# lightkurve/lightkurve

Measured on AMD Instinct MI355X. Metric: frequencies*targets/sec (Lomb-Scargle, ls_method='fast' (reference default): extirpolation + FFT) + BLS periods*targets/sec; max-power rel-err, higher is better.
Workload: dtype f64

## Files before the change

lightkurve_amd/csrc/lsfast.hip:

```cpp
#include <cmath>
#include <cstdlib>
#include <type_traits>
#include <vector>

#include "lk_common.hpp"
#include "ls_epilogue.hpp"

namespace lk {

typedef double lk_d2v __attribute__((ext_vector_type(2)));

constexpr int SPREAD_W = 1024;
constexpr int SPREAD_WW = 256;

struct FastStats {
    double wsum, ybar, YY, t0;
    double yws;
    double wmax;
    double vmax;
};

__device__ __forceinline__ void cadence_weights(const double *__restrict__ y, const double *__restrict__ dy, int64_t i,
                                                double wsum, double ybar, double &w, double &wy) {
    const double d = dy ? dy[i] : 1.0;
// ... 479 lines not shown
        }
        if (gout)
            gout[((size_t)blockIdx.y << (m1 + m2)) + ((((size_t)(c >> twl) << m1) + k1) << twl) + (c & (tw - 1))] = cmul(v, w);
        else
            G[(size_t)k1 * N2 + c] = cmul(v, w);
        w = cmul(w, step);
    };
    block_fft<LA, LB, 1>(CT, lds2, load, store);
}

constexpr int PRUNED_CT = 16;

constexpr int LSF_CHUNK_HALF_GB = 3;

template <int LP>
__global__ __launch_bounds__(PRUNED_CT * (1 << ((LP + 1) / 2)), 2) void fft_cols_pruned_kernel(
    const double2 *__restrict__ grids, int m1, int m2, const int *__restrict__ rows_used, double2 *__restrict__ gout,
    const double *__restrict__ t, const double *__restrict__ y, const double *__restrict__ dy,
    const int64_t *__restrict__ n_off, const FastStats *__restrict__ stats, int b0, double f0, double df, int fit_mean,
    const int *__restrict__ tab16, int ntab16) {
    extern __shared__ __attribute__((aligned(16))) double2 lds2[];
    constexpr int LA = (LP + 1) / 2, LB = LP / 2, A = 1 << LA, Bq = 1 << LB, P = 1 << LP, LDT = Bq + 1, FST = A * LDT + 1;
    constexpr int CT = PRUNED_CT, NT = CT * A;
    const int N1 = 1 << m1, N2 = 1 << m2, Q = N1 >> LP;
    const double2 *G = grids + ((size_t)blockIdx.y << (m1 + m2));
    const size_t tstride = (size_t)CT << m1, gstride = (size_t)(N2 / CT) * tstride;
    double2 *O = gout + (size_t)blockIdx.y * gstride + (size_t)blockIdx.x * tstride;
    const int c0 = blockIdx.x * CT;
    const int lbt = blockIdx.y / 3, g = blockIdx.y % 3;
    const int ru = rows_used[lbt * 4 + g];
    const int tid = threadIdx.x;
    const int f = tid % CT, jk = tid / CT;
    const bool p1 = jk < Bq, p2 = jk < A;
    const double invN1 = 1.0 / (double)N1, invN = 1.0 / (double)((size_t)1 << (m1 + m2));
    double2 xin[A];
    if (tab16 != nullptr && rows_used[lbt * 4 + 3]) {
        double2 *acc = lds2;
        for (int e = tid; e < ru * CT; e += NT) acc[e] = make_double2(0.0, 0.0);
        __syncthreads();
        if (!(g == 1 && !fit_mean)) {
            const int b = b0 + lbt;
            const int64_t lo = n_off[b];
            const FastStats st = stats[b];
            const double fac = g == 2 ? 2.0 : 1.0, dff = df * fac, f0f = f0 * fac, dn = (double)((size_t)1 << (m1 + m2));
            const int nfft = 1 << (m1 + m2);
            const int *tlo = tab16 + ((size_t)b * 4 + (g == 2 ? 2 : 0)) * ntab16, *thi = tlo + ntab16;
            const int S = g == 2 ? 4 : 8, rpi = 64 / S;
            const int lane = tid & 63, wv = tid >> 6, rr = lane / S, k = lane - rr * S;
            const int rpw = (ru + NT / 64 - 1) / (NT / 64);
            const int r_end = min(ru, (wv + 1) * rpw);
            auto visit = [&](int r, double ti, double yi, double di) {
                const double tt = ti - st.t0;
                const double wi = (1.0 / (di * di)) / st.wsum, wyi = wi * (yi - st.ybar);
                double c = 1.0, sn = 0.0;
                if (f0f > 0.0) phase_factor(f0f, tt, c, sn);
                const double xp = tt * dn * dff;
                const Stencil4 sp = stencil4(xp < dn ? xp : fmod(xp, dn), nfft);
                const double amp = g == 0 ? wyi : wi, ar = amp * c, ai = amp * sn;
                const int cbase = (r << m2) + c0;
#pragma unroll
                for (int q = 0; q < 4; ++q) {
                    const unsigned col = (unsigned)(sp.i0 + q - cbase);
                    if (q < sp.n && col < (unsigned)CT) {
                        unsafeAtomicAdd(&acc[r * CT + col].x, ar * sp.wt[q]);
                        unsafeAtomicAdd(&acc[r * CT + col].y, ai * sp.wt[q]);
                    }
                }
            };
            constexpr int UN = 4;
            for (int rb = wv * rpw; rb < r_end; rb += UN * rpi) {
                int ii[UN], ih[UN];
#pragma unroll
                for (int u = 0; u < UN; ++u) {
                    const int r = rb + u * rpi + rr;
                    const int blk = (min(r, r_end - 1) << (m2 - 4)) + blockIdx.x;
                    ii[u] = tlo[blk] + k;
                    ih[u] = thi[blk + 1];
                }
#pragma unroll
                for (int u = 0; u < UN; ++u) {
                    asm volatile("" : "+v"(ii[u]), "+v"(ih[u]));
                    if (rb + u * rpi + rr >= r_end) ii[u] = ih[u] = 0;
                }
                double tv[UN], yv[UN], dv[UN];
#pragma unroll
                for (int u = 0; u < UN; ++u) {
                    const bool ok = ii[u] < ih[u];
                    const int64_t ix = lo + (ok ? ii[u] : 0);
                    tv[u] = t[ix];
                    yv[u] = y[ix];
                    dv[u] = dy ? dy[ix] : 1.0;
                }
#pragma unroll
                for (int u = 0; u < UN; ++u) {
                    const int r = rb + u * rpi + rr;
                    if (ii[u] < ih[u]) visit(r, tv[u], yv[u], dv[u]);
                    int i = ii[u] + S;
                    while (__any(i < ih[u])) {
                        if (i < ih[u]) visit(r, t[lo + i], y[lo + i], dy ? dy[lo + i] : 1.0);
                        i += S;
                    }
                }
            }
        }
        __syncthreads();
        if (p1) {
#pragma unroll
            for (int i = 0; i < A; ++i) {
                const int r = i * Bq + jk;
                xin[i] = r < ru ? acc[r * CT + f] : make_double2(0.0, 0.0);
            }
        }
        __syncthreads();
    } else if (p1) {
#pragma unroll
        for (int i = 0; i < A; ++i) {
            const int r = i * Bq + jk;
            xin[i] = r < ru ? G[(size_t)r * N2 + c0 + f] : make_double2(0.0, 0.0);
        }
    }
    auto root = [](double x) {
        double sn, cs;
        sincospi(2.0 * x, &sn, &cs);
        return make_double2(cs, sn);
    };
    const double2 wj = root((double)jk * invN1), wq = root((double)Bq * invN1);
    const double2 tw_j = root((double)jk / (double)P);
    const double2 wc = root((double)(c0 + f) * invN), stepc = root((double)((long long)(c0 + f) * Q * A) * invN);
    double2 wjs = make_double2(1.0, 0.0), wqs = wjs;
    double2 wout = root((double)((long long)(c0 + f) * Q * jk) * invN);
    for (int s = 0; s < Q; ++s) {
        if (p1) {
            double2 v[A];
            if (s == 0) {
#pragma unroll
                for (int i = 0; i < A; ++i) v[i] = xin[i];
            } else {
                double2 w = wjs;
#pragma unroll
                for (int i = 0; i < A; ++i) {
                    v[i] = cmul(xin[i], w);
                    w = cmul(w, wqs);
                }
            }
            reg_fft<LA>(v);
            double2 w = make_double2(1.0, 0.0);
            double2 *row = lds2 + (size_t)f * FST + jk;
#pragma unroll
            for (int ka = 0; ka < A; ++ka) {
                row[ka * LDT] = cmul(v[brev_c(ka, LA)], w);
                w = cmul(w, tw_j);
            }
        }
        __syncthreads();
        if (p2) {
            const double2 *row = lds2 + (size_t)f * FST + (size_t)jk * LDT;
            double2 u[Bq];
#pragma unroll
            for (int j = 0; j < Bq; ++j) u[j] = row[j];
            reg_fft<LB>(u);
            double2 w = wout;
#pragma unroll
            for (int kb = 0; kb < Bq; ++kb) {
                const int q = jk + A * kb;
                O[(size_t)(Q * q + s) * CT + f] = cmul(u[brev_c(kb, LB)], w);
                w = cmul(w, stepc);
            }
        }
        wjs = cmul(wjs, wj);
        wqs = cmul(wqs, wq);
        wout = cmul(wout, wc);
        __syncthreads();
    }
}

template <int LA, int LB>
__global__ __launch_bounds__(256) void fft_rows_reg_kernel(const double2 *__restrict__ grids, int m1, int RT, int nkeep,
                                                            double2 *__restrict__ spec) {
    extern __shared__ __attribute__((aligned(16))) double2 lds2[];
    constexpr int m2 = LA + LB;
    const int N2 = 1 << m2;
    const double2 *G = grids + ((size_t)blockIdx.y << (m1 + m2));
    double2 *S = spec + (size_t)blockIdx.y * nkeep;
    const int r0 = blockIdx.x * RT;
    auto load = [&](int f, int c) -> double2 { return G[(size_t)(r0 + f) * N2 + c]; };
    auto store = [&](int f, int k2, double2 v, int) {
        const long long k = (long long)(r0 + f) + ((long long)k2 << m1);
        if (k < nkeep) S[k] = v;
    };
    block_fft<LA, LB, 0>(RT, lds2, load, store);
}

struct PeakPart {
    double v;
    long long k;
};

__device__ __forceinline__ bool peak_better(double v2, long long k2, double v, long long k) {
    return k2 >= 0 && (k < 0 || v2 > v || (v2 == v && k2 < k));
}

template <int LA, int LB, int KB>
__global__ __launch_bounds__(512) void fft_rows_power_kernel(const double2 *__restrict__ grids, int m1, int RT,
                                                              const int64_t *__restrict__ n_off,
                                                              const FastStats *__restrict__ stats, int b0, double f0,
                                                              double df, int64_t M, int fit_mean, int norm,
                                                              const double *__restrict__ scale,
                                                              double *__restrict__ power, int tw,
                                                              PeakPart *__restrict__ peaks) {
    extern __shared__ __attribute__((aligned(16))) double2 lds2[];
    constexpr int m2 = LA + LB, A = 1 << LA;
    const int N2 = 1 << m2;
    const int twl = tw ? 31 - __clz(tw) : 0;
    const size_t tstride = tw ? ((size_t)tw << m1) : 0, gstride = (size_t)1 << (m1 + m2);
    const int lb = blockIdx.y, r0 = blockIdx.x * RT;
    double2 keep0[KB], keep1[KB], keep2[KB];
#pragma unroll
    for (int q = 0; q < KB; ++q) keep0[q] = keep1[q] = keep2[q] = make_double2(0.0, 0.0);
    auto transform = [&](int g, double2(&keep)[KB]) {
        const double2 *G = grids + (size_t)(lb * 3 + g) * gstride;
        auto load = [&](int f, int c) -> double2 {
            return tw ? G[(size_t)(c >> twl) * tstride + ((size_t)(r0 + f) << twl) + (c & (tw - 1))] : G[(size_t)(r0 + f) * N2 + c];
        };
        auto store = [&](int, int, double2 v, int kb) {
            if (kb < KB) keep[kb < KB ? kb : 0] = v;
        };
        if (tw)
            block_fft<LA, LB, 2>(RT, lds2, load, store, tw);
        else
            block_fft<LA, LB, 0>(RT, lds2, load, store);
    };
    transform(0, keep0);
    __syncthreads();
    if (fit_mean) transform(1, keep1);
    __syncthreads();
    transform(2, keep2);
    const int tid = threadIdx.x;
    double best_v = 0.0;
    long long best_k = -1;
    if (tid < RT * A) {
        const int ka = tid / RT, f = tid - ka * RT;
        const int b = b0 + lb;
        const FastStats st = stats[b];
        const double nn = (double)(n_off[b + 1] - n_off[b]);
        const double sc = scale ? scale[b] : 1.0;
        const int k1 = r0 + f;
        const double twopi = 6.283185307179586;
        double ph_c = 1.0, ph_s = 0.0, st_c = 1.0, st_s = 0.0;
        if (st.t0 != 0.0) {
            const long long kfirst = (long long)k1 + ((long long)ka << m1);
            sincos(twopi * st.t0 * (f0 + df * (double)kfirst), &ph_s, &ph_c);
            sincos(twopi * st.t0 * (df * (double)((long long)A << m1)), &st_s, &st_c);
        }
#pragma unroll
        for (int kb = 0; kb < KB; ++kb) {
            const long long k = (long long)k1 + ((long long)(ka + A * kb) << m1);
            if (k < M) {
                double2 a = keep0[kb], bq = keep1[kb], c2 = keep2[kb];
                if (st.t0 != 0.0) {
                    const double c = ph_c, s = ph_s;
                    a = make_double2(a.x * c - a.y * s, a.x * s + a.y * c);
                    bq = make_double2(bq.x * c - bq.y * s, bq.x * s + bq.y * c);
                    const double cc = c * c - s * s, ss = 2.0 * s * c;
                    c2 = make_double2(c2.x * cc - c2.y * ss, c2.x * ss + c2.y * cc);
                }
                const double pw = gls_power_sums(a.y, a.x, bq.y, bq.x, c2.y, c2.x, fit_mean, norm, st.YY, 0.5 * st.wsum, nn, sc);
                power[(size_t)b * (size_t)M + k] = pw;
                if (pw == pw && peak_better(pw, k, best_v, best_k)) {
                    best_v = pw;
                    best_k = k;
                }
            }
            const double nc = ph_c * st_c - ph_s * st_s, ns = ph_s * st_c + ph_c * st_s;
            ph_c = nc;
            ph_s = ns;
        }
    }
    if (peaks == nullptr) return;
#pragma unroll
    for (int o = 32; o > 0; o >>= 1) {
        const double v2 = __shfl_xor(best_v, o);
        const long long k2 = __shfl_xor(best_k, o);
        if (peak_better(v2, k2, best_v, best_k)) {
            best_v = v2;
            best_k = k2;
        }
    }
    if ((tid & 63) == 0)
        peaks[((size_t)lb * gridDim.x + blockIdx.x) * (blockDim.x >> 6) + (tid >> 6)] = PeakPart{best_v, best_k};
}

__device__ __forceinline__ double dpp_ror8(double x) {
    int lo = __double2loint(x), hi = __double2hiint(x);
    lo = __builtin_amdgcn_update_dpp(0, lo, 0x128, 0xF, 0xF, true);
    hi = __builtin_amdgcn_update_dpp(0, hi, 0x128, 0xF, 0xF, true);
    return __hiloint2double(hi, lo);
}

struct Rows512 {
    static constexpr int RT = 8;
    static constexpr int SK = 34;
    static constexpr int SF = 16 * SK + 4;
    static constexpr int NT = RT * 32;
    static constexpr size_t LDS_BYTES = (size_t)RT * SF * 8;
};

__global__ __launch_bounds__(Rows512::NT, 2) void fft_rows512_power_kernel(
    const double2 *__restrict__ grids, int m1, int ntargets, const int64_t *__restrict__ n_off,
    const FastStats *__restrict__ stats, int b0, double f0, double df, int64_t M, int fit_mean, int norm,
    const double *__restrict__ scale, double *__restrict__ power, PeakPart *__restrict__ peaks) {
    using R = Rows512;
    constexpr int RT = R::RT, SK = R::SK, SF = R::SF;
    extern __shared__ __attribute__((aligned(16))) double tile512[];
    const int tid = threadIdx.x;
    const size_t gstride = (size_t)1 << (m1 + 9);
    const int tiles_per_target = (1 << m1) / RT;
    const int jl = tid & 15, f1 = (tid >> 4) & (RT - 1), jh = tid >> 7, j = jl + 16 * jh;
    const int f2 = tid & 7, e = (tid >> 3) & 1, ka = tid >> 4;
    auto tile_base = [&](int T) {
        const int lbT = ntargets - 1 - T / tiles_per_target, r0T = (T % tiles_per_target) * RT;
        return grids + (size_t)lbT * 3 * gstride + ((size_t)jh << (m1 + 4)) + ((size_t)(r0T + f1) << 4) + jl;
    };
    double2 v[16];
    auto load = [&](const double2 *G) {
#pragma unroll
        for (int i = 0; i < 16; ++i) {
            const lk_d2v q = __builtin_nontemporal_load(reinterpret_cast<const lk_d2v *>(G + ((size_t)i << (m1 + 5))));
            v[i] = make_double2(q.x, q.y);
        }
    };
    double2 step1, step4;
    {
        double s, c;
        sincospi((double)j * (1.0 / 256.0), &s, &c);
        step1 = make_double2(c, s);
        sincospi((double)j * (1.0 / 64.0), &s, &c);
        step4 = make_double2(c, s);
    }
    double2 keep[3][4];
    double *row1 = tile512 + f1 * SF + j;
    const double *row2 = tile512 + f2 * SF + ka * SK + e;
    auto process = [&](auto Gc, auto refill) {
        constexpr int G = decltype(Gc)::value;
        __builtin_amdgcn_sched_barrier(0);
        reg_fft<4>(v);
        __builtin_amdgcn_sched_barrier(0);
        {
            double2 w = step1;
#pragma unroll
            for (int bb = 1; bb < 4; ++bb) {
#pragma unroll
                for (int a = 0; a < 4; ++a) v[brev_c(4 * a + bb, 4)] = cmul(v[brev_c(4 * a + bb, 4)], w);
                if (bb < 3) w = cmul(w, step1);
            }
        }
        __builtin_amdgcn_sched_barrier(0);
        {
            double2 w = step4;
#pragma unroll
            for (int a = 1; a < 4; ++a) {
#pragma unroll
                for (int bb = 0; bb < 4; ++bb) v[brev_c(4 * a + bb, 4)] = cmul(v[brev_c(4 * a + bb, 4)], w);
                if (a < 3) w = cmul(w, step4);
            }
        }
        __builtin_amdgcn_sched_barrier(0);
        double ure[16], uim[16];
#pragma unroll
        for (int k = 0; k < 16; ++k) row1[k * SK] = v[brev_c(k, 4)].x;
        __syncthreads();
#pragma unroll
        for (int jj = 0; jj < 16; ++jj) ure[jj] = row2[2 * jj];
        __syncthreads();
#pragma unroll
        for (int k = 0; k < 16; ++k) row1[k * SK] = v[brev_c(k, 4)].y;
        __builtin_amdgcn_sched_barrier(0);
        refill();
        __syncthreads();
#pragma unroll
        for (int jj = 0; jj < 16; ++jj) uim[jj] = row2[2 * jj];
        __builtin_amdgcn_sched_barrier(0);
        double2 s0[8], s1[8];
#pragma unroll
        for (int q = 0; q < 8; ++q) {
            s0[q] = make_double2(ure[2 * q], uim[2 * q]);
            s1[q] = make_double2(ure[2 * q + 1], uim[2 * q + 1]);
        }
        reg_fft<3>(s0);
        __builtin_amdgcn_sched_barrier(0);
        reg_fft<3>(s1);
        __builtin_amdgcn_sched_barrier(0);
        auto pval = [&](int kb) -> double2 {
            const double2 a = s0[brev_c(kb, 3)], bq = s1[brev_c(kb, 3)];
            double2 hsum;
            if (kb == 0)
                hsum = make_double2(a.x + bq.x, a.y + bq.y);
            else if (kb == 4)
                hsum = make_double2(a.x - bq.y, a.y + bq.x);
            else
                hsum = make_double2(a.x + (bq.x * R32C[2 * kb] - bq.y * R32S[2 * kb]),
                                    a.y + (bq.x * R32S[2 * kb] + bq.y * R32C[2 * kb]));
            if (kb == 0) return hsum;
            const double wc = e ? R32C[kb] : 1.0, ws = e ? R32S[kb] : 0.0;
            return make_double2(hsum.x * wc - hsum.y * ws, hsum.x * ws + hsum.y * wc);
        };
#pragma unroll
        for (int q = 0; q < 4; ++q) {
            const double2 plo = pval(q), phi = pval(q + 4);
            const double2 mine = e ? phi : plo, send = e ? plo : phi;
            keep[G][q] = make_double2(mine.x + dpp_ror8(send.x), mine.y + dpp_ror8(send.y));
            __builtin_amdgcn_sched_barrier(0);
        }
    };
    using I0 = std::integral_constant<int, 0>;
    using I1 = std::integral_constant<int, 1>;
    using I2 = std::integral_constant<int, 2>;
    const int T = blockIdx.x;
    const double2 *Gt = tile_base(T);
    load(Gt);
    {
        const int lb = ntargets - 1 - T / tiles_per_target, r0 = (T % tiles_per_target) * RT;
        process(I0{}, [&] { load(Gt + gstride); });
        __syncthreads();
        process(I1{}, [&] { load(Gt + 2 * gstride); });
        __syncthreads();
        process(I2{}, [] {});
        double best_v = 0.0;
        long long best_k = -1;
        {
            const int b = b0 + lb;
            const FastStats st = stats[b];
            const double nn = (double)(n_off[b + 1] - n_off[b]);
            const double sc = scale ? scale[b] : 1.0;
            const int k1 = r0 + f2;
            const double twopi = 6.283185307179586;
            double ph_c = 1.0, ph_s = 0.0, st_c = 1.0, st_s = 0.0;
            if (st.t0 != 0.0) {
                const long long kfirst = (long long)k1 + ((long long)(ka + 64 * e) << m1);
                sincos(twopi * st.t0 * (f0 + df * (double)kfirst), &ph_s, &ph_c);
                sincos(twopi * st.t0 * (df * (double)((long long)16 << m1)), &st_s, &st_c);
            }
#pragma unroll 1
            for (int q = 0; q < 4; ++q) {
                const long long k = (long long)k1 + ((long long)(ka + 16 * (4 * e + q)) << m1);
                if (k < M) {
                    double2 a = keep[0][0], bq = keep[1][0], c2 = keep[2][0];
                    if (st.t0 != 0.0) {
                        const double c = ph_c, s = ph_s;
                        a = make_double2(a.x * c - a.y * s, a.x * s + a.y * c);
                        bq = make_double2(bq.x * c - bq.y * s, bq.x * s + bq.y * c);
                        const double cc = c * c - s * s, ss = 2.0 * s * c;
                        c2 = make_double2(c2.x * cc - c2.y * ss, c2.x * ss + c2.y * cc);
                    }
                    const double pw = gls_power_sums(a.y, a.x, bq.y, bq.x, c2.y, c2.x, fit_mean, norm, st.YY, 0.5 * st.wsum, nn, sc);
                    power[(size_t)b * (size_t)M + k] = pw;
                    if (pw == pw && peak_better(pw, k, best_v, best_k)) {
                        best_v = pw;
                        best_k = k;
                    }
                }
                const double nc = ph_c * st_c - ph_s * st_s, ns = ph_s * st_c + ph_c * st_s;
                ph_c = nc;
                ph_s = ns;
#pragma unroll
                for (int g = 0; g < 3; ++g)
#pragma unroll
                    for (int r = 0; r < 3; ++r) keep[g][r] = keep[g][r + 1];
            }
        }
        if (peaks != nullptr) {
#pragma unroll
            for (int o = 32; o > 0; o >>= 1) {
                const double v2 = __shfl_xor(best_v, o);
                const long long k2 = __shfl_xor(best_k, o);
                if (peak_better(v2, k2, best_v, best_k)) {
                    best_v = v2;
                    best_k = k2;
                }
            }
            if ((tid & 63) == 0)
                peaks[((size_t)lb * tiles_per_target + (T % tiles_per_target)) * (R::NT / 64) + (tid >> 6)] = PeakPart{best_v, best_k};
        }
    }
}

__global__ __launch_bounds__(64) void lsf_peaks_kernel(const PeakPart *__restrict__ peaks, int nparts, int b0,
                                                        double *__restrict__ max_out, int64_t *__restrict__ arg_out) {
    const PeakPart *pp = peaks + (size_t)blockIdx.x * nparts;
    double v = 0.0;
    long long k = -1;
    for (int i = threadIdx.x; i < nparts; i += 64)
        if (peak_better(pp[i].v, pp[i].k, v, k)) {
            v = pp[i].v;
            k = pp[i].k;
        }
#pragma unroll
    for (int o = 32; o > 0; o >>= 1) {
        const double v2 = __shfl_xor(v, o);
        const long long k2 = __shfl_xor(k, o);
        if (peak_better(v2, k2, v, k)) {
            v = v2;
            k = k2;
        }
    }
    if (threadIdx.x == 0) {
        max_out[b0 + blockIdx.x] = k >= 0 ? v : NAN;
        arg_out[b0 + blockIdx.x] = (int64_t)k;
    }
}

__global__ __launch_bounds__(256) void lsf_scatter_multi_kernel(const double *__restrict__ t, const double *__restrict__ y,
                                                                 const double *__restrict__ dy,
                                                                 const int64_t *__restrict__ n_off,
                                                                 const FastStats *__restrict__ stats, int b0, double f0,
                                                                 double df, int nfft, int nterms,
                                                                 double2 *__restrict__ grids) {
    const int b = b0 + blockIdx.y;
    const int64_t lo = n_off[b];
    const int n = (int)(n_off[b + 1] - lo);
    const int i = blockIdx.x * 256 + threadIdx.x;
    if (i >= n) return;
    const FastStats st = stats[b];
    const double tt = t[lo + i] - st.t0;
    double2 *g0 = grids + (size_t)blockIdx.y * 3 * nterms * nfft;
    double wi, wyi;
    cadence_weights(y, dy, lo + i, st.wsum, st.ybar, wi, wyi);
    const Quantum Qy = make_quantum(st.vmax), Qw = make_quantum(st.wmax);
    for (int fac = 1; fac <= 2 * nterms; ++fac) {
        const double dff = df * (double)fac, f0f = f0 * (double)fac;
        double c = 1.0, s = 0.0;
        if (f0f > 0.0) phase_factor(f0f, tt, c, s);
        const Stencil4 sp = stencil4(fmod(tt * (double)nfft * dff, (double)nfft), nfft);
        extirpolate4(g0 + (size_t)(nterms + fac - 1) * nfft, sp, wi * c, wi * s, Qw);
        if (fac <= nterms) extirpolate4(g0 + (size_t)(fac - 1) * nfft, sp, wyi * c, wyi * s, Qy);
    }
}

template <int NT>
__global__ __launch_bounds__(256) void lsf_chi2_power_kernel(const double2 *__restrict__ spec,
                                                              const int64_t *__restrict__ n_off,
                                                              const FastStats *__restrict__ stats, int b0, double f0,
                                                              double df, int64_t M, int fit_mean, int norm,
                                                              const double *__restrict__ scale,
                                                              double *__restrict__ power) {
    const int b = b0 + blockIdx.y;
    const int64_t j = (int64_t)blockIdx.x * 256 + threadIdx.x;
    if (j >= M) return;
    const FastStats st = stats[b];
    const double2 *s0 = spec + (size_t)blockIdx.y * 3 * NT * M;
    Chi2Sums<NT> sums;
    const double twopi = 6.283185307179586;
#pragma unroll
    for (int m = 1; m <= 2 * NT; ++m) {
        double cph = 1.0, sph = 0.0;
        if (st.t0 != 0.0) sincos(twopi * st.t0 * (double)m * (f0 + df * (double)j), &sph, &cph);
        const double2 a = s0[(size_t)(NT + m - 1) * M + j];
        sums.Cw[m - 1] = a.x * cph - a.y * sph;
        sums.Sw[m - 1] = a.x * sph + a.y * cph;
        if (m <= NT) {
            const double2 y = s0[(size_t)(m - 1) * M + j];
            sums.Cy[m - 1] = y.x * cph - y.y * sph;
            sums.Sy[m - 1] = y.x * sph + y.y * cph;
        }
    }
    const double n = (double)(n_off[b + 1] - n_off[b]);
    power[(size_t)b * (size_t)M + j] =
        chi2_normalise(sums.solve_lu(st.yws, fit_mean), norm, st.YY, 0.5 * st.wsum, n, scale ? scale[b] : 1.0);
}

__global__ __launch_bounds__(256) void lsf_power_kernel(const double2 *__restrict__ spec,
                                                         const int64_t *__restrict__ n_off,
                                                         const FastStats *__restrict__ stats, int b0, double f0,
                                                         double df, int64_t M, int fit_mean, int norm,
                                                         const double *__restrict__ scale,
                                                         double *__restrict__ power) {
    const int b = b0 + blockIdx.y;
    const int64_t j = (int64_t)blockIdx.x * 256 + threadIdx.x;
    if (j >= M) return;
    const FastStats st = stats[b];
    const double2 *s0 = spec + (size_t)blockIdx.y * 3 * M;
    double2 a = s0[j], bq = s0[M + j], c2 = s0[2 * M + j];
    if (st.t0 != 0.0) {
        const double twopi = 6.283185307179586;
        double s, c;
        sincos(twopi * st.t0 * (f0 + df * (double)j), &s, &c);
        a = make_double2(a.x * c - a.y * s, a.x * s + a.y * c);
        bq = make_double2(bq.x * c - bq.y * s, bq.x * s + bq.y * c);
        sincos(twopi * st.t0 * (2.0 * f0 + 2.0 * df * (double)j), &s, &c);
        c2 = make_double2(c2.x * c - c2.y * s, c2.x * s + c2.y * c);
    }
    const double n = (double)(n_off[b + 1] - n_off[b]);
    power[(size_t)b * (size_t)M + j] = gls_power_sums(a.y, a.x, bq.y, bq.x, c2.y, c2.x, fit_mean, norm, st.YY,
                                                      0.5 * st.wsum, n, scale ? scale[b] : 1.0);
}

__global__ __launch_bounds__(256) void lsf_unquantize_kernel(double2 *__restrict__ grids, int m1, int m2,
                                                              const int *__restrict__ rows_used,
                                                              const FastStats *__restrict__ stats, int b0, int ngp, int n_wy) {
    const int lbt = blockIdx.y / ngp, g = blockIdx.y % ngp;
    if (rows_used && rows_used[lbt * 4 + 3]) return;
    const int ru = rows_used ? rows_used[lbt * 4 + g] : (1 << m1);
    const FastStats st = stats[b0 + lbt];
    const double q = make_quantum(g < n_wy ? st.vmax : st.wmax).q;
    if (!(q > 0.0)) return;
    const int N2 = 1 << m2;
    double2 *G = grids + ((size_t)blockIdx.y << (m1 + m2));
    for (int r = blockIdx.x * 8; r < min(blockIdx.x * 8 + 8, ru); ++r)
        for (int c = threadIdx.x; c < N2; c += 256) {
            const double2 v = G[(size_t)r * N2 + c];
            G[(size_t)r * N2 + c] = make_double2((double)__double_as_longlong(v.x) * q, (double)__double_as_longlong(v.y) * q);
        }
}

__global__ __launch_bounds__(256) void lsf_zero_kernel(double2 *__restrict__ grids, int m1, int m2,
                                                        const int *__restrict__ rows_used) {
    if (rows_used[(blockIdx.y / 3) * 4 + 3]) return;
    const int ru = rows_used[(blockIdx.y / 3) * 4 + (blockIdx.y % 3)];
    const int N2 = 1 << m2;
    double2 *G = grids + ((size_t)blockIdx.y << (m1 + m2));
    for (int r = blockIdx.x * 8; r < min(blockIdx.x * 8 + 8, ru); ++r)
        for (int c = threadIdx.x; c < N2; c += 256) G[(size_t)r * N2 + c] = make_double2(0.0, 0.0);
}

constexpr int COLS_TILE_PTS = 4096;

template <int LA, int LB>
static void launch_cols_t(lk_handle *h, int m2, int ngrids, double2 *grids, const int *rows_used, double2 *gout, int tw,
                          hipStream_t stream) {
    constexpr int A = 1 << LA, Bq = 1 << LB, n = A * Bq, LDT = Bq + 1, FST = A * LDT + 1;
    const int N2 = 1 << m2;
    const int CT = std::max(1, std::min(N2, std::min(COLS_TILE_PTS / n, 256 / std::max(A, Bq))));
    const int nt = ((CT * std::max(A, Bq) + 63) / 64) * 64;
    (void)want_lds(h, reinterpret_cast<const void *>(fft_cols_reg_kernel<LA, LB>), 160 * 1024);
    hipLaunchKernelGGL((fft_cols_reg_kernel<LA, LB>), dim3(N2 / CT, ngrids), dim3(nt), (size_t)CT * FST * 16, stream, grids,
                       m2, CT, rows_used, gout, tw);
}

static int tile_width(int m1, int m2) {
    const int la1 = (m1 + 1) / 2, lb1 = m1 / 2, n1 = 1 << m1;
    const int ct = std::max(1, std::min(1 << m2, std::min(COLS_TILE_PTS / n1, 256 / std::max(1 << la1, 1 << lb1))));
    const int bq2 = 1 << (m2 / 2);
    return std::min(ct, bq2);
}

template <int LA, int LB>
static void launch_rows_t(lk_handle *h, int m1, int ngrids, const double2 *grids, int nkeep, double2 *spec, hipStream_t stream) {
    constexpr int A = 1 << LA, Bq = 1 << LB, n = A * Bq, LDT = Bq + 1, FST = A * LDT + 1;
    const int N1 = 1 << m1;
    const int RT = std::max(1, std::min(N1, std::min(4096 / n, 256 / std::max(A, Bq))));
    const int nt = ((RT * std::max(A, Bq) + 63) / 64) * 64;
    (void)want_lds(h, reinterpret_cast<const void *>(fft_rows_reg_kernel<LA, LB>), 100 * 1024);
    hipLaunchKernelGGL((fft_rows_reg_kernel<LA, LB>), dim3(N1 / RT, ngrids), dim3(nt), (size_t)RT * FST * 16, stream,
                       grids, m1, RT, nkeep, spec);
}

struct FusedArgs {
    const int64_t *n_off;
    const FastStats *stats;
    int b0;
    double f0, df;
    int64_t M;
    int fit_mean, norm;
    const double *scale;
    double *power;
    PeakPart *peaks;
};

template <int LA, int LB>
static int rows_power_rt(int m1) {
    constexpr int A = 1 << LA, Bq = 1 << LB, n = A * Bq;
    return std::max(1, std::min(1 << m1, std::min(4096 / n, 256 / std::max(A, Bq))));
}

template <int LA, int LB, int KB>
static void launch_rows_power_t(lk_handle *h, int m1, int ntargets, const double2 *grids, const FusedArgs &a, int tw,
                                hipStream_t stream) {
    constexpr int A = 1 << LA, Bq = 1 << LB, LDT = Bq + 1, FST = A * LDT + 1;
    const int N1 = 1 << m1;
    const int RT = rows_power_rt<LA, LB>(m1);
    const int nt = ((RT * std::max(A, Bq) + 63) / 64) * 64;
    (void)want_lds(h, reinterpret_cast<const void *>(fft_rows_power_kernel<LA, LB, KB>), 160 * 1024);
    hipLaunchKernelGGL((fft_rows_power_kernel<LA, LB, KB>), dim3(N1 / RT, ntargets), dim3(nt), (size_t)RT * FST * 16,
                       stream, grids, m1, RT, a.n_off, a.stats, a.b0, a.f0, a.df, a.M, a.fit_mean, a.norm, a.scale,
                       a.power, tw, a.peaks);
}

static bool rows_power_available(int m1, int m2, int64_t M) {
    const int LA = (m2 + 1) / 2, Aa = 1 << LA;
    const long long k2need = (M + ((long long)1 << m1) - 1) >> m1;
    return m2 >= 4 && m2 <= 10 && (k2need + Aa - 1) / Aa <= 8;
}

#define LK_M2_SWITCH(m2, X) \
    switch (m2) {           \
        case 4: X(2, 2)     \
        case 5: X(3, 2)     \
        case 6: X(3, 3)     \
        case 7: X(4, 3)     \
        case 8: X(4, 4)     \
        case 9: X(5, 4)     \
        default: X(5, 5)    \
    }

static int rows_power_parts(int m1, int m2) {
#define LK_X(la, lb)                                                                                   \
    {                                                                                                  \
        const int rt = rows_power_rt<la, lb>(m1);                                                      \
        return ((1 << m1) / rt) * ((rt * std::max(1 << (la), 1 << (lb)) + 63) / 64);                   \
    }
    LK_M2_SWITCH(m2, LK_X)
#undef LK_X
}

static bool rows512_applies(int m1, int m2, int64_t M, int tw) {
    const long long k2need = (M + ((long long)1 << m1) - 1) >> m1;
    return m2 == 9 && tw == PRUNED_CT && m1 >= 3 && k2need <= 128;
}

static void launch_rows512(lk_handle *h, int m1, int ntargets, const double2 *grids, const FusedArgs &a, hipStream_t stream) {
    const int ntiles = ((1 << m1) / Rows512::RT) * ntargets;
    hipLaunchKernelGGL(fft_rows512_power_kernel, dim3(ntiles), dim3(Rows512::NT), Rows512::LDS_BYTES, stream, grids, m1, ntargets,
                       a.n_off, a.stats, a.b0, a.f0, a.df, a.M, a.fit_mean, a.norm, a.scale, a.power, a.peaks);
}

static bool launch_rows_power(lk_handle *h, int m1, int m2, int ntargets, const double2 *grids, const FusedArgs &a, int tw,
                              hipStream_t stream) {
    const int LA = (m2 + 1) / 2, Aa = 1 << LA;
    const long long k2need = (a.M + ((long long)1 << m1) - 1) >> m1;
    if (rows512_applies(m1, m2, a.M, tw)) {
        launch_rows512(h, m1, ntargets, grids, a, stream);
        return true;
    }
    const int kb = (int)((k2need + Aa - 1) / Aa);
    if (kb > 8 || m2 < 4 || m2 > 10) return false;
#define LK_X(la, lb)                                                            \
    {                                                                           \
        if (kb <= 4)                                                            \
            launch_rows_power_t<la, lb, 4>(h, m1, ntargets, grids, a, tw, stream); \
        else                                                                    \
            launch_rows_power_t<la, lb, 8>(h, m1, ntargets, grids, a, tw, stream); \
        return true;                                                            \
    }
    LK_M2_SWITCH(m2, LK_X)
#undef LK_X
}

static void launch_cols_reg(lk_handle *h, int m1, int m2, int ngrids, double2 *grids, const int *rows_used, double2 *gout,
                            int tw, hipStream_t stream) {
#define LK_X(la, lb)                                                                  \
    {                                                                                 \
        launch_cols_t<la, lb>(h, m2, ngrids, grids, rows_used, gout, tw, stream);      \
        break;                                                                        \
    }
    LK_M2_SWITCH(m1, LK_X)
#undef LK_X
}

static void launch_rows_reg(lk_handle *h, int m1, int m2, int ngrids, const double2 *grids, int nkeep, double2 *spec,
                            hipStream_t stream) {
#define LK_X(la, lb)                                                          \
    {                                                                         \
        launch_rows_t<la, lb>(h, m1, ngrids, grids, nkeep, spec, stream);      \
        break;                                                                \
    }
    LK_M2_SWITCH(m2, LK_X)
#undef LK_X
}

__global__ __launch_bounds__(256) void lsf_plan_kernel(const int *__restrict__ rows_used, int B, int *__restrict__ plan) {
    int mx = 0, unordered = 0;
    for (int b = threadIdx.x; b < B; b += 256) {
        mx = max(mx, max(rows_used[b * 4], max(rows_used[b * 4 + 1], rows_used[b * 4 + 2])));
        unordered += rows_used[b * 4 + 3] ? 0 : 1;
    }
    __shared__ int smx[256], sun[256];
    smx[threadIdx.x] = mx;
    sun[threadIdx.x] = unordered;
    __syncthreads();
    for (int s = 128; s > 0; s >>= 1) {
        if ((int)threadIdx.x < s) {
            smx[threadIdx.x] = max(smx[threadIdx.x], smx[threadIdx.x + s]);
            sun[threadIdx.x] += sun[threadIdx.x + s];
        }
        __syncthreads();
    }
    if (threadIdx.x == 0) {
        plan[0] = smx[0];
        plan[1] = sun[0];
    }
}

struct SpreadArgs {
    const double *t, *y, *dy;
    const int64_t *n_off;
    const FastStats *stats;
    int b0;
    double f0, df;
    int fit_mean;
    const int *tab16;
    int ntab16;
};

template <int LP>
static void launch_cols_pruned_t(lk_handle *h, int m1, int m2, int ngrids, const double2 *grids, const int *rows_used,
                                 double2 *gout, const SpreadArgs &sa, hipStream_t stream) {
    constexpr int LA = (LP + 1) / 2, LB = LP / 2, A = 1 << LA, Bq = 1 << LB, LDT = Bq + 1, FST = A * LDT + 1;
    (void)want_lds(h, reinterpret_cast<const void *>(fft_cols_pruned_kernel<LP>), 160 * 1024);
    hipLaunchKernelGGL((fft_cols_pruned_kernel<LP>), dim3((1 << m2) / PRUNED_CT, ngrids), dim3(PRUNED_CT * A),
                       (size_t)PRUNED_CT * FST * 16, stream, grids, m1, m2, rows_used, gout, sa.t, sa.y, sa.dy, sa.n_off,
                       sa.stats, sa.b0, sa.f0, sa.df, sa.fit_mean, sa.tab16, sa.ntab16);
}

static bool launch_cols_pruned(lk_handle *h, int lp, int m1, int m2, int ngrids, const double2 *grids, const int *rows_used,
                               double2 *gout, const SpreadArgs &sa, hipStream_t stream) {
    switch (lp) {
        case 5: launch_cols_pruned_t<5>(h, m1, m2, ngrids, grids, rows_used, gout, sa, stream); return true;
        case 6: launch_cols_pruned_t<6>(h, m1, m2, ngrids, grids, rows_used, gout, sa, stream); return true;
        case 7: launch_cols_pruned_t<7>(h, m1, m2, ngrids, grids, rows_used, gout, sa, stream); return true;
        case 8: launch_cols_pruned_t<8>(h, m1, m2, ngrids, grids, rows_used, gout, sa, stream); return true;
        default: return false;
    }
}

static int ilog2_ceil(long long v) {
    int m = 0;
    while (((long long)1 << m) < v) ++m;
    return m;
}

int lsfast_launch(lk_handle *h, int B, const int64_t *n_off_host, const double *t, const double *y, const double *dy,
                  double f0, double df, int64_t M, int fit_mean, int center_data, int normalization,
                  const double *scale, int oversampling, double *power, hipStream_t stream, double *max_out,
                  int64_t *arg_out) {
    LK_REQUIRE(B >= 0 && n_off_host != nullptr, "bad batch description");
    LK_REQUIRE(M >= 0, "M must be >= 0");
    if (B == 0 || M == 0) return LK_OK;
    LK_REQUIRE(t && y && power, "t, y, power must be non-NULL");
    LK_REQUIRE((max_out == nullptr) == (arg_out == nullptr), "max_power and argmax must both be given (or both NULL)");
    LK_REQUIRE(normalization >= LK_NORM_STANDARD && normalization <= LK_NORM_LK_PSD, "unknown normalization %d",
               normalization);
    LK_REQUIRE(f0 >= 0.0, "Frequencies must be positive");
    LK_REQUIRE(df > 0.0, "Frequency steps must be positive");
    LK_REQUIRE(oversampling >= 1 && oversampling <= 64, "oversampling outside 1..64");
    LK_REQUIRE(n_off_host[0] == 0, "n_off[0] must be 0");
    int64_t nmax = 0;
    for (int b = 0; b < B; ++b) {
        const int64_t n = n_off_host[b + 1] - n_off_host[b];
        LK_REQUIRE(n >= 1 && n < ((int64_t)1 << 30), "target %d has %lld cadences", b, (long long)n);
        nmax = std::max(nmax, n);
    }
    const int m = std::max(3, ilog2_ceil((long long)M * oversampling));
    LK_REQUIRE(m <= 24, "FFT grid 2^%d too large (M = %lld)", m, (long long)M);
    const int nfft = 1 << m, m1 = (m + 1) / 2, m2 = m / 2;
    const int N1 = 1 << m1, N2 = 1 << m2;
    const int CT = std::max(1, std::min(N2, 4096 / N1)), RT = std::max(1, std::min(N1, 4096 / N2));
    const size_t chunk_bytes = (size_t)LSF_CHUNK_HALF_GB << 29;
    int Bc = (int)std::max<size_t>(1, std::min<size_t>((size_t)B, chunk_bytes / ((size_t)48 * nfft)));
    if (Bc >= 8) Bc &= ~3;
    const bool reg_path = m1 >= 4 && m1 <= 10 && m2 >= 4 && m2 <= 10;
    const bool fused = reg_path && rows_power_available(m1, m2, M);
    const int nparts512 = (m2 == 9) ? (N1 / 8) * 4 : 0;
    const int nparts_gen = fused ? rows_power_parts(m1, m2) : 0;
    const int nparts_max = std::max(nparts512, nparts_gen);
    const int ntab256 = (nfft + SPREAD_WW - 1) / SPREAD_WW + 3;
    const int ntab16 = (m2 >= 8 && m2 <= 10) ? (int)((((size_t)256 << m2) >> 4) + 3) : 0;
    const int ntab_max = std::max(ntab256, ntab16);
    h->ws.reset();
    int rc = h->ws.reserve((size_t)(B + 1) * 8 + (size_t)B * sizeof(FastStats) + 512 +
                           (size_t)Bc * 3 * nfft * 16 * 2 + (size_t)Bc * 3 * M * 16 + (size_t)B * 16 +
                           (size_t)B * 4 * ntab_max * 4 + (size_t)(B + 1) * nparts_max * sizeof(PeakPart) + 16384);
    if (rc) return rc;
    int64_t *d_off = (int64_t *)h->ws.alloc((size_t)(B + 1) * 8);
    FastStats *d_stats = (FastStats *)h->ws.alloc((size_t)B * sizeof(FastStats));
    double2 *d_grids = (double2 *)h->ws.alloc((size_t)Bc * 3 * nfft * 16);
    double2 *d_spec = fused ? nullptr : (double2 *)h->ws.alloc((size_t)Bc * 3 * M * 16);
    rc = h->stage.copy(d_off, n_off_host, (size_t)(B + 1) * 8, stream);
    if (rc) return rc;
    const int tw = tile_width(m1, m2);
    double2 *d_grids2 = fused ? (double2 *)h->ws.alloc((size_t)Bc * 3 * nfft * 16) : nullptr;
    LK_REQUIRE(!fused || d_grids2 != nullptr, "workspace exhausted");
    int *d_rows = (int *)h->ws.alloc((size_t)B * 4 * 4);
    int *d_plan = (int *)h->ws.alloc(64);
    int *d_tab = reg_path ? (int *)h->ws.alloc((size_t)B * 4 * ntab_max * 4) : nullptr;
    PeakPart *d_peaks = (fused && max_out) ? (PeakPart *)h->ws.alloc((size_t)B * nparts_max * sizeof(PeakPart)) : nullptr;
    hipLaunchKernelGGL(lsf_prep_kernel, dim3(B), dim3(PREP_NT), 0, stream, t, y, dy, d_off, (fit_mean || center_data) ? 1 : 0,
                       d_stats, df, nfft, m2, d_rows);
    int lp = 0, n_unordered = B, spread_blocks = (nfft + SPREAD_W - 1) / SPREAD_W;
    if (fused) {
        if (!h->h_plan) LK_HIP_CHECK(hipHostMalloc(reinterpret_cast<void **>(&h->h_plan), 64, hipHostMallocDefault));
        hipLaunchKernelGGL(lsf_plan_kernel, dim3(1), dim3(256), 0, stream, d_rows, B, d_plan);
        LK_HIP_CHECK(hipMemcpyAsync(h->h_plan, d_plan, 8, hipMemcpyDeviceToHost, stream));
        LK_HIP_CHECK(hipStreamSynchronize(stream));
        n_unordered = h->h_plan[1];
        spread_blocks = std::min(spread_blocks, (int)((((size_t)std::max(1, h->h_plan[0]) << m2) + SPREAD_W - 1) / SPREAD_W));
        if (m2 >= 8 && m2 <= 10 && N2 >= PRUNED_CT) {
            const int want = std::max(5, ilog2_ceil(std::max(1, h->h_plan[0])));
            if (want <= 8 && want < m1) lp = want;
        }
    }
    const int ntab = lp ? ntab16 : ntab256;
    if (reg_path && n_unordered < B)
        hipLaunchKernelGGL(lsf_tables_kernel, dim3((unsigned)((nmax + 256 * TAB_PER_LANE - 1) / (256 * TAB_PER_LANE)), B), dim3(256), 0, stream, t, d_off, d_stats,
                           d_rows, df, nfft, m2, lp ? 4 : 8, d_tab, ntab);
    if (!reg_path) {
        (void)want_lds(h, reinterpret_cast<const void *>(fft_cols_kernel), 100 * 1024);
        (void)want_lds(h, reinterpret_cast<const void *>(fft_rows_kernel), 100 * 1024);
    }
    const size_t ldsA = ((size_t)CT * N1 + N1 / 2 + 1) * 16, ldsB = ((size_t)RT * N2 + N2 / 2 + 1) * 16;
    const bool two_streams = fused && lp != 0 && n_unordered == 0 && B > Bc;
    if (two_streams) {
        if (!h->ev_ls_fork) LK_HIP_CHECK(hipEventCreateWithFlags(&h->ev_ls_fork, hipEventDisableTiming));
        LK_HIP_CHECK(hipEventRecord(h->ev_ls_fork, stream));
        if (!h->s_ls_aux[0]) LK_HIP_CHECK(hipStreamCreateWithFlags(&h->s_ls_aux[0], hipStreamNonBlocking));
        if (!h->ev_ls_join[0]) LK_HIP_CHECK(hipEventCreateWithFlags(&h->ev_ls_join[0], hipEventDisableTiming));
        LK_HIP_CHECK(hipStreamWaitEvent(h->s_ls_aux[0], h->ev_ls_fork, 0));
    }
    hipStream_t caller_stream = stream;
    struct AuxGuard {
        hipStream_t aux;
        ~AuxGuard() {
            if (aux) (void)hipStreamSynchronize(aux);
        }
    } aux_guard{two_streams ? h->s_ls_aux[0] : nullptr};
    int chunk_no = 0;
    for (int b0 = 0; b0 < B; b0 += Bc, ++chunk_no) {
        const int nb = std::min(Bc, B - b0);
        double2 *gr = d_grids;
        const bool on_aux = two_streams && (chunk_no & 1);
        stream = on_aux ? h->s_ls_aux[0] : caller_stream;
        double2 *inter = on_aux ? d_grids : d_grids2;
        if (!reg_path) {
            LK_HIP_CHECK(hipMemsetAsync(gr, 0, (size_t)nb * 3 * nfft * 16, stream));
        } else if (n_unordered > 0) {
            hipLaunchKernelGGL(lsf_zero_kernel, dim3((N1 + 7) / 8, nb * 3), dim3(256), 0, stream, gr, m1, m2,
                               d_rows + (size_t)b0 * 4);
        }
        if (!reg_path || n_unordered > 0) {
            hipLaunchKernelGGL(lsf_scatter_kernel, dim3((unsigned)((nmax + 255) / 256), nb), dim3(256), 0, stream, t, y,
                               dy, d_off, d_stats, b0, f0, df, nfft, fit_mean, gr,
                               reg_path ? d_rows + (size_t)b0 * 4 : (const int *)nullptr);
            hipLaunchKernelGGL(lsf_unquantize_kernel, dim3((N1 + 7) / 8, nb * 3), dim3(256), 0, stream, gr, m1, m2,
                               reg_path ? d_rows + (size_t)b0 * 4 : (const int *)nullptr, d_stats, b0, 3, 1);
        }
        if (reg_path && !lp && n_unordered < B)
            hipLaunchKernelGGL(lsf_spread_owner_kernel, dim3((unsigned)spread_blocks, nb, 2), dim3(256), 0, stream, t, y, dy,
                               d_off, d_stats, b0, f0, df, nfft, m2, fit_mean, gr, d_rows + (size_t)b0 * 4, d_tab, ntab);
        if (fused) {
            const int nparts = rows512_applies(m1, m2, M, lp ? PRUNED_CT : tw) ? nparts512 : nparts_gen;
            const FusedArgs fa{d_off, d_stats, b0, f0, df, M, fit_mean, normalization, scale, power,
                               d_peaks ? d_peaks + (size_t)b0 * nparts : nullptr};
            if (lp) {
                const SpreadArgs sa{t, y, dy, d_off, d_stats, b0, f0, df, fit_mean, n_unordered < B ? d_tab : nullptr, ntab};
                LK_REQUIRE(launch_cols_pruned(h, lp, m1, m2, nb * 3, gr, d_rows + (size_t)b0 * 4, inter, sa, stream),
                           "no pruned column kernel for 2^%d rows", lp);
            } else {
                launch_cols_reg(h, m1, m2, nb * 3, gr, d_rows + (size_t)b0 * 4, inter, tw, stream);
            }
            LK_REQUIRE(launch_rows_power(h, m1, m2, nb, inter, fa, lp ? PRUNED_CT : tw, stream),
                       "no step-2 kernel for this layout");
            if (b0 + nb == B) {
                if (two_streams) {
                    LK_HIP_CHECK(hipEventRecord(h->ev_ls_join[0], h->s_ls_aux[0]));
                    LK_HIP_CHECK(hipStreamWaitEvent(caller_stream, h->ev_ls_join[0], 0));
                }
                aux_guard.aux = nullptr;
                stream = caller_stream;
                if (d_peaks)
                    hipLaunchKernelGGL(lsf_peaks_kernel, dim3(B), dim3(64), 0, stream, d_peaks, nparts, 0, max_out, arg_out);
            }
            continue;
        }
        if (reg_path) {
            launch_cols_reg(h, m1, m2, nb * 3, gr, d_rows + (size_t)b0 * 4, nullptr, 1, stream);
            launch_rows_reg(h, m1, m2, nb * 3, gr, (int)M, d_spec, stream);
        } else {
            hipLaunchKernelGGL(fft_cols_kernel, dim3(N2 / CT, nb * 3), dim3(256), ldsA, stream, gr, m1, m2, CT);
            hipLaunchKernelGGL(fft_rows_kernel, dim3(N1 / RT, nb * 3), dim3(256), ldsB, stream, gr, m1, m2, RT,
                               (int)M, d_spec);
        }
        hipLaunchKernelGGL(lsf_power_kernel, dim3((unsigned)((M + 255) / 256), nb), dim3(256), 0, stream, d_spec,
                           d_off, d_stats, b0, f0, df, M, fit_mean, normalization, scale, power);
    }
    stream = caller_stream;
    if (const int lrc = take_lds_error(h)) return lrc;
    LK_HIP_CHECK(hipGetLastError());
    if (max_out && !fused) return argmax_launch(h, B, M, power, max_out, arg_out, stream);
    return LK_OK;
}

int lsfastchi2_launch(lk_handle *h, int B, const int64_t *n_off_host, const double *t, const double *y, const double *dy,
                      double f0, double df, int64_t M, int nterms, int fit_mean, int center_data, int normalization,
                      const double *scale, int oversampling, double *power, hipStream_t stream) {
    LK_REQUIRE(nterms >= 1 && nterms <= LK_MAX_NTERMS, "nterms must be between 1 and %d (got %d)", LK_MAX_NTERMS, nterms);
    if (nterms == 1)
        return lsfast_launch(h, B, n_off_host, t, y, dy, f0, df, M, fit_mean, center_data, normalization, scale,
                             oversampling, power, stream, nullptr, nullptr);
    if (nterms > 4)
        return ls_chi2_launch(h, B, n_off_host, t, y, dy, nullptr, f0, df, M, nterms, fit_mean, center_data, normalization, scale,
                              power, stream);
    LK_REQUIRE(B >= 0 && n_off_host != nullptr, "bad batch description");
    LK_REQUIRE(M >= 0, "M must be >= 0");
    if (B == 0 || M == 0) return LK_OK;
    LK_REQUIRE(t && y && power, "t, y, power must be non-NULL");
    LK_REQUIRE(f0 >= 0.0, "Frequencies must be positive");
    LK_REQUIRE(df > 0.0, "Frequency steps must be positive");
    LK_REQUIRE(oversampling >= 1, "oversampling must be >= 1");
    LK_REQUIRE(normalization >= LK_NORM_STANDARD && normalization <= LK_NORM_LK_PSD, "unknown normalization %d",
               normalization);
    LK_REQUIRE(n_off_host[0] == 0, "n_off[0] must be 0");
    int64_t nmax = 0;
    for (int b = 0; b < B; ++b) {
        const int64_t n = n_off_host[b + 1] - n_off_host[b];
        LK_REQUIRE(n >= 1 && n < ((int64_t)1 << 30), "target %d has %lld cadences", b, (long long)n);
        nmax = std::max(nmax, n);
    }
    const int m = ilog2_ceil((long long)oversampling * (long long)M);
    LK_REQUIRE(m >= 2 && m <= 24, "FFT grid of 2^%d points is outside the supported range (2^2 .. 2^24: the in-LDS column\n"
               "transform of longer grids does not fit 160 KB)", m);
    const int nfft = 1 << m, m1 = (m + 1) / 2, m2 = m / 2;
    const int N1 = 1 << m1, N2 = 1 << m2;
    const int NG = 3 * nterms;
    const size_t per_target = (size_t)NG * nfft * 16;
    const int Bc = (int)std::max<size_t>(1, std::min<size_t>((size_t)B, ((size_t)2 << 30) / per_target));
    h->ws.reset();
// ... 51 lines not shown
```

Baseline: 9.440 billion.

## Make rows512 power kernel persistent with LDS-parked results and prefetch of next tile

Turns the rows512 FFT+power kernel into a persistent kernel that launches about two workgroups per CU and loops over tiles. Before the power epilogue runs, it issues the global loads for the next tile so memory latency overlaps with power computation. The first two FFT stages' results are parked in extra LDS instead of registers, which cuts register pressure. A DPP exchange reorders outputs so each lane walks frequencies in interleaved order, and the loop exits early once no lane has a valid k. The cost is more LDS per block (with a request to raise the LDS limit), an extra barrier per tile, and more complex phase-rotation bookkeeping.

New measurement: 9.388 billion. About the same (-0.5%).

```diff
diff --git a/lightkurve_amd/csrc/lsfast.hip b/lightkurve_amd/csrc/lsfast.hip
--- a/lightkurve_amd/csrc/lsfast.hip
+++ b/lightkurve_amd/csrc/lsfast.hip
@@ -805,7 +805,8 @@
     static constexpr int SK = 34;
     static constexpr int SF = 16 * SK + 4;
     static constexpr int NT = RT * 32;
-    static constexpr size_t LDS_BYTES = (size_t)RT * SF * 8;
+    static constexpr size_t TILE_BYTES = (size_t)RT * SF * 8;
+    static constexpr size_t LDS_BYTES = TILE_BYTES + (size_t)8 * NT * 16;
 };
 
 __global__ __launch_bounds__(Rows512::NT, 2) void fft_rows512_power_kernel(
@@ -840,7 +841,8 @@
         sincospi((double)j * (1.0 / 64.0), &s, &c);
         step4 = make_double2(c, s);
     }
-    double2 keep[3][4];
+    double2 keep2[4];
+    double2 *park = reinterpret_cast<double2 *>(tile512 + RT * SF) + tid;
     double *row1 = tile512 + f1 * SF + j;
     const double *row2 = tile512 + f2 * SF + ka * SK + e;
     auto process = [&](auto Gc, auto refill) {
@@ -907,21 +909,34 @@
             const double wc = e ? R32C[kb] : 1.0, ws = e ? R32S[kb] : 0.0;
             return make_double2(hsum.x * wc - hsum.y * ws, hsum.x * ws + hsum.y * wc);
         };
+        double2 own[4];
 #pragma unroll
         for (int q = 0; q < 4; ++q) {
             const double2 plo = pval(q), phi = pval(q + 4);
             const double2 mine = e ? phi : plo, send = e ? plo : phi;
-            keep[G][q] = make_double2(mine.x + dpp_ror8(send.x), mine.y + dpp_ror8(send.y));
+            own[q] = make_double2(mine.x + dpp_ror8(send.x), mine.y + dpp_ror8(send.y));
             __builtin_amdgcn_sched_barrier(0);
         }
+        const double2 sa = e ? own[0] : own[1], sb = e ? own[2] : own[3];
+        const double2 ra = make_double2(dpp_ror8(sa.x), dpp_ror8(sa.y)), rb = make_double2(dpp_ror8(sb.x), dpp_ror8(sb.y));
+        auto put = [&](int q, double2 x) {
+            if constexpr (G < 2)
+                park[(G * 4 + q) * R::NT] = x;
+            else
+                keep2[q] = x;
+        };
+        put(0, e ? ra : own[0]);
+        put(1, e ? rb : own[2]);
+        put(2, e ? own[1] : ra);
+        put(3, e ? own[3] : rb);
     };
     using I0 = std::integral_constant<int, 0>;
     using I1 = std::integral_constant<int, 1>;
     using I2 = std::integral_constant<int, 2>;
-    const int T = blockIdx.x;
-    const double2 *Gt = tile_base(T);
+    const int ntiles = tiles_per_target * ntargets;
+    const double2 *Gt = tile_base(blockIdx.x);
     load(Gt);
-    {
+    for (int T = blockIdx.x; T < ntiles; T += gridDim.x) {
         const int lb = ntargets - 1 - T / tiles_per_target, r0 = (T % tiles_per_target) * RT;
         process(I0{}, [&] { load(Gt + gstride); });
         __syncthreads();
@@ -937,17 +952,39 @@
             const double sc = scale ? scale[b] : 1.0;
             const int k1 = r0 + f2;
             const double twopi = 6.283185307179586;
-            double ph_c = 1.0, ph_s = 0.0, st_c = 1.0, st_s = 0.0;
+            double ph_c = 1.0, ph_s = 0.0, st_c = 1.0, st_s = 0.0, ph4_c = 1.0, ph4_s = 0.0;
+            auto rotate = [&] {
+                const double nc = ph_c * st_c - ph_s * st_s, ns = ph_s * st_c + ph_c * st_s;
+                ph_c = nc;
+                ph_s = ns;
+            };
+            auto chain_head = [&](int kb0) {
+                const long long kfirst = (long long)k1 + ((long long)(ka + 16 * kb0) << m1);
+                sincos(twopi * st.t0 * (f0 + df * (double)kfirst), &ph_s, &ph_c);
+                const double c0 = ph_c, s0 = ph_s;
+                rotate();
+                ph_c = e ? ph_c : c0;
+                ph_s = e ? ph_s : s0;
+            };
             if (st.t0 != 0.0) {
-                const long long kfirst = (long long)k1 + ((long long)(ka + 64 * e) << m1);
-                sincos(twopi * st.t0 * (f0 + df * (double)kfirst), &ph_s, &ph_c);
                 sincos(twopi * st.t0 * (df * (double)((long long)16 << m1)), &st_s, &st_c);
+                chain_head(4);
+                ph4_c = ph_c;
+                ph4_s = ph_s;
+                chain_head(0);
             }
+            __builtin_amdgcn_sched_barrier(0);
+            if (T + (int)gridDim.x < ntiles) {
+                Gt = tile_base(T + (int)gridDim.x);
+                load(Gt);
+            }
+            __builtin_amdgcn_sched_barrier(0);
 #pragma unroll 1
             for (int q = 0; q < 4; ++q) {
-                const long long k = (long long)k1 + ((long long)(ka + 16 * (4 * e + q)) << m1);
+                const long long k = (long long)k1 + ((long long)(ka + 16 * (2 * q + e)) << m1);
+                if (!__any(k < M)) break;
                 if (k < M) {
-                    double2 a = keep[0][0], bq = keep[1][0], c2 = keep[2][0];
+                    double2 a = park[q * R::NT], bq = park[(4 + q) * R::NT], c2 = keep2[0];
                     if (st.t0 != 0.0) {
                         const double c = ph_c, s = ph_s;
                         a = make_double2(a.x * c - a.y * s, a.x * s + a.y * c);
@@ -962,13 +999,17 @@
                         best_k = k;
                     }
                 }
-                const double nc = ph_c * st_c - ph_s * st_s, ns = ph_s * st_c + ph_c * st_s;
-                ph_c = nc;
-                ph_s = ns;
-#pragma unroll
-                for (int g = 0; g < 3; ++g)
-#pragma unroll
-                    for (int r = 0; r < 3; ++r) keep[g][r] = keep[g][r + 1];
+                if (st.t0 != 0.0) {
+                    if (q == 1) {
+                        ph_c = ph4_c;
+                        ph_s = ph4_s;
+                    } else {
+                        rotate();
+                        rotate();
+                    }
+                }
+#pragma unroll
+                for (int r = 0; r < 3; ++r) keep2[r] = keep2[r + 1];
             }
         }
         if (peaks != nullptr) {
@@ -984,6 +1025,7 @@
             if ((tid & 63) == 0)
                 peaks[((size_t)lb * tiles_per_target + (T % tiles_per_target)) * (R::NT / 64) + (tid >> 6)] = PeakPart{best_v, best_k};
         }
+        __syncthreads();
     }
 }
 
@@ -1221,8 +1263,9 @@
 }
 
 static void launch_rows512(lk_handle *h, int m1, int ntargets, const double2 *grids, const FusedArgs &a, hipStream_t stream) {
-    const int ntiles = ((1 << m1) / Rows512::RT) * ntargets;
-    hipLaunchKernelGGL(fft_rows512_power_kernel, dim3(ntiles), dim3(Rows512::NT), Rows512::LDS_BYTES, stream, grids, m1, ntargets,
+    const int ntiles = ((1 << m1) / Rows512::RT) * ntargets, nwg = std::min(ntiles, 2 * h->num_cu);
+    (void)want_lds(h, reinterpret_cast<const void *>(fft_rows512_power_kernel), 160 * 1024);
+    hipLaunchKernelGGL(fft_rows512_power_kernel, dim3(nwg), dim3(Rows512::NT), Rows512::LDS_BYTES, stream, grids, m1, ntargets,
                        a.n_off, a.stats, a.b0, a.f0, a.df, a.M, a.fit_mean, a.norm, a.scale, a.power, a.peaks);
 }
 
```
